# Yachim/schwarzschild-raytracer

Hardware: AMD Instinct MI355X
Metric: Mpixels/s at 1920x1080, 2000 geodesic steps; 1/2/4/8 MI355X (higher is better)
Workload: dtype f32

## Files before the change

schwarzschild-raytracer_amd/csrc/device_scene.h:

```cpp
#ifndef SR_DEVICE_SCENE_H
#define SR_DEVICE_SCENE_H

#include <stdint.h>

#include "sr/sr.h"

#define SR_OBJ_FLOATS 120

#define SR_F_POS 0
#define SR_F_AXES 3
#define SR_F_P0 12
#define SR_F_BOX_FACE0 16
#define SR_F_FACE_STRIDE 14

#define SR_KIND_EXACT 0
#define SR_KIND_BUDGET 1
#define SR_KIND_CHORD 2
#define SR_MU_PLANAR 1.0e-4f
#define SR_MU_QUADRATIC 2.0e-3f
#define SR_CYL_QMARGIN 4.0e-6f
#ifndef SR_BUDGET_DPMIN
#define SR_BUDGET_DPMIN 0.02f
#endif
#ifndef SR_BUDGET_TMAX
// ... 16 lines not shown
    float pl1;
    float f[SR_OBJ_FLOATS - 4];
} sr_dev_obj;

typedef struct {
    int32_t type;
    int32_t cyl;
    float rb, mp, br, mu, pl1;
    float qk;
    float bc[3], x0;
    float pos[3], x1;
    float a0[3], x2;
    float a1[3], rf;
    float a2[3], cn;
} sr_dev_slot;

#define SR_PS_HITS 4
#define SR_PS_FIELDS (4 + 8 * SR_PS_HITS + 16)
#define SR_OPQ_RADIUS 2

#define SR_SEG_FLOATS 16
#define SR_TR_BLOCK 8
#define SR_TR_GROUP 8
#define SR_TR_BLOCKS ((SR_MAX_POINTS - 1 + SR_TR_BLOCK - 1) / SR_TR_BLOCK)
#define SR_TR_GROUPS ((SR_TR_BLOCKS + SR_TR_GROUP - 1) / SR_TR_GROUP)
#define SR_TR_BOUND_FLOATS 12
#define SR_SEGS_BUF_FLOATS ((SR_MAX_POINTS - 1) * SR_SEG_FLOATS + (SR_TR_BLOCKS + SR_TR_GROUPS) * SR_TR_BOUND_FLOATS)

typedef struct {
    int32_t num_objects;
// ... 92 lines not shown
```

schwarzschild-raytracer_amd/csrc/kernels/geodesic.hip:

```cpp
#include <hip/hip_runtime.h>

#include <cstdint>
#include <type_traits>

typedef float sr_v4f __attribute__((ext_vector_type(4)));
typedef const __attribute__((address_space(4))) sr_v4f sr_cfloat4;
__device__ __forceinline__ float4 ldc(const sr_cfloat4* p) {
    const sr_v4f v = *p;
    return make_float4(v.x, v.y, v.z, v.w);
}

#include "../device_scene.h"

namespace {

#define SR_PI 3.1415926535f
#define SR_EPS 0.0000001f

struct f2 { float x, y; };
struct f3 { float x, y, z; };
struct f4 { float x, y, z, w; };
struct m3 { f3 c0, c1, c2; };

__device__ __forceinline__ f2 F2(float x, float y) { f2 r; r.x = x; r.y = y; return r; }
// ... 306 lines not shown
    const float th0 = __builtin_fmaf(kap, len, __builtin_fmaf(2.0f * perr, il, 1e-4f));
    const float m = (sl.mp + sl.mu * __builtin_fmaf(3.1f, a, 1.0f)) * 1.001f + perr;
    const float R = fabsf(y) - m;
    if (!(R > 0.0f)) return 0.0f;
    const float b = c + th0;
    const float L = (__builtin_amdgcn_sqrtf(__builtin_fmaf(b, b, 2.0f * kap * R)) - b) * (a2 * (1.0f / 6.06f));
    const float ch = 1.5f * a * dphi;
    const float Lc = fminf(L, fminf(__builtin_fmaf(0.5f, a, -ch), (1.5f - th0) * (a2 * (1.0f / 6.06f)) - ch));
    const float th1 = __builtin_fmaf(kap, Lc, th0);
    const float f = 1.0f - (th1 * th1 + th1 * th0 + th0 * th0) * (1.0f / 6.0f);
    return (Lc > 0.0f && f > 0.0f) ? Lc * f * 0.998f : 0.0f;
}
#ifndef SR_INIT_WINDOW
#define SR_INIT_WINDOW 1
#endif
__device__ __forceinline__ float plane_window_start(const sr_dev_slot& sl, f3 A, f3 d, float a, float perr, float dphi) {
    const f3 nrm_ = ld3(sl.a1);
    const float y = dot(A - ld3(sl.pos), nrm_);
    if (!(a > 1.0f)) return 0.0f;
    const float a2 = a * a;
    const float kap = 6.06f * __builtin_amdgcn_rcpf(a2);
    const float c = (y > 0.0f ? -1.0f : 1.0f) * dot(d, nrm_);
    const float th0 = 1e-4f;
    const float m = (sl.mp + sl.mu * __builtin_fmaf(3.1f, a, 1.0f)) * 1.001f + perr;
    const float R = fabsf(y) - m;
    if (!(R > 0.0f)) return 0.0f;
    const float b = c + th0;
    const float L = (__builtin_amdgcn_sqrtf(__builtin_fmaf(b, b, 2.0f * kap * R)) - b) * (a2 * (1.0f / 6.06f));
    const float ch = 1.5f * a * dphi;
    const float Lc = fminf(L, fminf(__builtin_fmaf(0.5f, a, -ch), (1.5f - th0) * (a2 * (1.0f / 6.06f)) - ch));
    const float th1 = __builtin_fmaf(kap, Lc, th0);
    const float f = 1.0f - (th1 * th1 + th1 * th0 + th0 * th0) * (1.0f / 6.0f);
    return (Lc > 0.0f && f > 0.0f) ? Lc * f * 0.998f : 0.0f;
}
#ifndef SR_OUT_CYL_CM
#define SR_OUT_CYL_CM 1
#endif
#ifndef SR_OUT_FAR
#define SR_OUT_FAR 1
#endif
__device__ __forceinline__ bool outward_slot(const sr_dev_slot& sl, bool cyl_par, float a, float dip) {
    if (SR_OUT_CYL_CM) cyl_par = false;
    if (sl.type == SR_OBJECT_PLANE || (sl.type == SR_OBJECT_CYLINDER && (cyl_par || !(sl.x1 > 0.0f)))) return false;
    if (SR_OUT_FAR)
        return outward_clear(sl.rf, 0.0f, slot_mu(sl), sl.type == SR_OBJECT_CYLINDER ? sl.qk : 0.0f, sl.pl1, a, dip);
// ... 118 lines not shown
    __device__ __forceinline__ void setMh(float v) const { st(L::BMH, v); }
    __device__ __forceinline__ uint32_t cm() const { return __float_as_uint(ld(L::BCM)) & 0xffu; }
    __device__ __forceinline__ uint32_t excl() const { return __float_as_uint(ld(L::BCM)) >> 8; }
    __device__ __forceinline__ void setCm(uint32_t cm, uint32_t excl) const {
        st(L::BCM, __uint_as_float(cm | (excl << 8)));
    }
    __device__ __forceinline__ float etr() const { return ld(L::BTR); }
    __device__ __forceinline__ void setEtr(float v) const { st(L::BTR, v); }
    __device__ __forceinline__ float uhi() const { return ld(L::BUHI); }
    __device__ __forceinline__ void setUhi(float v) const { st(L::BUHI, v); }
    static __device__ __forceinline__ bool inner(float uhi) { return uhi > SR_BH_U && uhi < 1.0f; }
    static __device__ __forceinline__ float ulo_of(float uhi, float u_f) { return inner(uhi) ? SR_BH_ULO2 : u_f; }
    SR_PROBE_BUDGET_FIELDS
};

__device__ __forceinline__ uint32_t xplane_bit(const sr_dev_slot& sl, int j, f3 n, float nn, float xs) {
    if (sl.type == SR_OBJECT_PLANE || sl.type == SR_OBJECT_CYLINDER) return 0u;
    const float h = dot(ld3(sl.bc), n);
    const float need = (sl.br + sl.mu * xs) * 1.001f + 1.0e-4f + 1.0e-5f * sl.cn;
    return (uint32_t)(h * h > (need * need) * (nn * 1.0002f)) << j;
}
#ifndef SR_XCYL
#define SR_XCYL 1
#endif
__device__ __forceinline__ uint32_t xcyl_bit(const sr_dev_slot& sl, int j, f3 n, float nn, float need) {
    const float h = dot(ld3(sl.bc), n);
    return (uint32_t)(h * h > (need * need) * (nn * 1.0002f)) << j;
}
__device__ __forceinline__ float orbit_e(float u, float du) {
    return u < 0.6f ? __builtin_fmaf(du, du, u * u * (1.0f - u)) : INFINITY;
}
#ifndef SR_XPERI
#define SR_XPERI 1
#endif
template <class BS>
__device__ __forceinline__ uint32_t budget_cyl_frame(const sr_dev_scene* __restrict__ sc, BS& bs, f3 nv, f3 tv) {
    uint32_t c = (uint32_t)sc->budget_cyl_mask;
    uint32_t cm = 0;
#pragma unroll
    for (int k = 0; k < BS::NC; k++) {
        if (c) {
            const f3 ax = ld3(sc->slots[__builtin_ctz(c)].a1);
// ... 24 lines not shown
    }
#endif
    bs.setCm(cm, x);
}

template <class BS>
__device__ __forceinline__ bool cyl_par_bit(const sr_dev_scene* __restrict__ sc, const BS& bs, int j) {
    const uint32_t cyl = (uint32_t)sc->budget_cyl_mask;
    if (!((cyl >> (j - 1)) & 1u)) return false;
    return (bs.cm() >> __builtin_popcount(cyl & ((1u << (j - 1)) - 1u))) & 1u;
}

__device__ float clearance_tr(const sr_dev_scene* __restrict__ sc, const float* __restrict__ segs, f3 A, bool outward,
                              float a, float dip, float rlen, uint32_t& gm);

template <bool START_WINDOW, class BS>
__device__ __forceinline__ void budget_init(const sr_dev_scene* __restrict__ sc, const float* __restrict__ segs,
                                            BS& bs, f3 A, f3 nv, f3 tv,
                                            bool outward, float dip, bool bh_ok, bool falling, float xs, float u2w,
                                            const float* xneed, const float* xperi, float eo, f3 d, float dphi) {
    const float a = __builtin_amdgcn_sqrtf(dot(A, A));
    const int nb = sc->num_budget;
    bs.setT(0.0f);
    bs.setC(dot(A, nv), dot(A, tv));
    const float m0 = 2.0e-6f * (a + 1.0f);
    float m = INFINITY;
    const uint32_t cm = budget_cyl_frame(sc, bs, nv, tv);
    bs.setCm(cm, 0u);
    const f3 xn = cross(nv, tv);
    const float xnn = dot(xn, xn);
    uint32_t xcl = 0;
    {
        float e = clearance_bh(a);
        float uhi = SR_U_NOWIN;
        if (SR_BH_WINDOW && bh_ok && a > SR_BH_RWIN) {
            e = INFINITY;
            uhi = SR_BH_U;
        }
        if (SR_BH_WINDOW2 && dip > SR_BH_DIP2 && a * u2w > 1.000001f && a < SR_BH_RMAX2 && (falling || !(a > SR_BH_RWIN))) {
            e = INFINITY;
            uhi = u2w;
        }
        bs.setUhi(uhi);
        if (outward && outward_clear(1.0f, 0.0f, SR_MU_QUADRATIC, 0.0f, 0.0f, a, dip)) e = INFINITY;
        e -= m0;
        bs.E[0] = e;
        m = nmin(m, e);
    }
    if constexpr (BS::TR) {
        uint32_t gm;
        const float e = clearance_tr(sc, segs, A, outward, a, dip, -1.0f, gm) - m0;
        bs.setEtr(e);
        m = nmin(m, e);
    }
    sr_dev_slot nxt;
    if (nb > 0) nxt = sc->slots[0];
#pragma unroll 1
    for (int j = 1; j <= nb; j++) {
        const sr_dev_slot sl = pin_slot(nxt);
        if (j < nb) nxt = sc->slots[j];
        if (SR_XPLANE) xcl |= xplane_bit(sl, j, xn, xnn, xs);
        if (SR_XCYL && eo <= SR_XCYL_EMAX) xcl |= xcyl_bit(sl, j, xn, xnn, xneed[j - 1]);
        if (SR_XPERI && eo <= xperi[j - 1]) xcl |= 1u << j;
        float e = clearance_obj(sl, A, a) - m0;
        if (START_WINDOW && SR_INIT_WINDOW && (sl.type == SR_OBJECT_RECTANGLE || sl.type == SR_OBJECT_DISK ||
                               sl.type == SR_OBJECT_HOLLOW_DISK || sl.type == SR_OBJECT_PLANE) &&
            sl.mp < INFINITY && e < 0.5f * a) {
            const float w = plane_window_start(sl, A, d, a, m0, dphi);
            e = w > e ? w : e;
        }
        if (outward && outward_slot(sl, cyl_par_bit(sc, bs, j), a, dip)) e = INFINITY;
        if ((xcl >> j) & 1u) e = INFINITY;
        bs.E[j * SR_E_STRIDE] = e;
        m = nmin(m, e);
    }
    bs.setCm(cm, xcl);
    bs.setM(m);
    float mh = INFINITY;
    uint32_t c = (uint32_t)sc->budget_cyl_mask;
#pragma unroll
    for (int k = 0; k < BS::NC; k++) {
        if (c) {
            const float e = clearance_slab(sc->slots[__builtin_ctz(c)], A, a) - m0;
            bs.E[(BS::L::SLAB0 + k) * SR_E_STRIDE] = e;
            mh = nmin(mh, e);
            c &= c - 1;
        }
    }
    bs.setMh(mh);
}

template <int NC>
struct CylDirs {
    float pa[NC > 0 ? NC : 1], pb[NC > 0 ? NC : 1];
};
template <class BS>
__device__ __forceinline__ CylDirs<BS::NC> cyl_dirs(const sr_dev_scene* __restrict__ sc, const BS& bs) {
    CylDirs<BS::NC> d;
// ... 940 lines not shown
        return F4(at(f, id), at(f + 1, id), at(f + 2, id), at(f + 3, id));
    }
};

__device__ __forceinline__ f4 crosshair_frag(const sr_dev_frame& fr, const Pix& q) {
    f4 frag = F4(0.0f, 0.0f, 0.0f, 0.0f);
    if (fr.crosshair) {
        f2 uv = F2((float)(2 * q.px + 1) / (float)fr.width - 1.0f, (float)(2 * q.py + 1) / (float)fr.height - 1.0f);
        float hx = fabsf(uv.x * fr.res_x / 2.0f), hy = fabsf(uv.y * fr.res_y / 2.0f);
        if ((hx < 1.0f && hy > 5.0f && hy < 15.0f) || (hy < 1.0f && hx > 5.0f && hx < 15.0f))
            frag = F4(0.5f, 0.5f, 0.5f, 0.5f);
    }
    return frag;
}

__device__ __forceinline__ int init_pixel(const sr_dev_frame& fr, const sr_dev_cam& cam, const Pix& q, Ray& r) {
    f2 uv = F2((float)(2 * q.px + 1) / (float)fr.width - 1.0f, (float)(2 * q.py + 1) / (float)fr.height - 1.0f);
    f2 uvv = F2(uv.x, uv.y * fr.res_y / fr.res_x);
    m3 axes = ldm(cam.axes);
    r.ro = ld3(cam.pos);
    r.rd = nrm(mv(axes, F3(uvv.x, uvv.y, cam.ray_forward)));
    r.nv = nrm(r.ro);
    r.steps = 0;
    r.i = 0;
    SR_PROBE(probe_ray_init(r));
    const bool flat = fr.raytrace_type == SR_RAYTRACE_FLAT ||
                      (fr.raytrace_type == SR_RAYTRACE_HALF_WIDTH && uv.x > 2.0f * fr.curved_percentage + -1.0f) ||
                      (fr.raytrace_type == SR_RAYTRACE_HALF_HEIGHT && uv.y > 2.0f * fr.curved_percentage + -1.0f);
    if (flat || fabsf(dot(r.rd, r.nv)) >= 1.0f - SR_EPS) return ST_FLAT;
    if (fr.percent_black >= 0.0f) {
        float x = t_sin(uvv.x * 12.9898f + uvv.y * 78.233f) * 43758.5453f;
        if (x - floorf(x) <= fr.percent_black) return ST_DONE;
    }
    r.tv = nrm(cross(cross(r.nv, r.rd), r.nv));
    r.u = 1.0f / len(r.ro);
    r.du = -r.u * dot(r.rd, r.nv) / dot(r.rd, r.tv);
    return -1;
}

__shared__ uint32_t sr_lds_pid[SR_WG];
struct HitLog {
    PS ps;
    int n;
    __device__ __forceinline__ uint32_t id() const {
        typedef volatile const __attribute__((address_space(3))) uint32_t lds_u32;
        uint32_t t = threadIdx.x;
        asm volatile("" : "+v"(t));
        return *(lds_u32*)&sr_lds_pid[t];
    }
};
// ... 20 lines not shown
    const float l4 = ddu(u + k3 * h);
    un = u + h6 * (__builtin_fmaf(2.0f, k3, __builtin_fmaf(2.0f, k2, k1)) + k4);
    dun = du + h6 * (__builtin_fmaf(2.0f, l3, __builtin_fmaf(2.0f, l2, l1)) + l4);
}

__device__ __forceinline__ bool flat_misses(const sr_dev_scene* __restrict__ sc, f3 ro, f3 rd) {
    return !sc->tr_visible && dot(ro, rd) >= 0.0f && dot(ro, ro) > sc->flat_miss_r2;
}

__shared__ int sr_lds_ev[SR_WG / 64];

template <bool CULL, bool RECORD, bool WCOST = false, int NB = SR_MAX_BUDGET, int FU = SR_FAST_UNROLL,
          int NC = SR_NC_KERNEL, bool TR = false>
__device__ __forceinline__ int integrate(const sr_dev_scene* __restrict__ sc, const float* __restrict__ segs,
                                         const float4* __restrict__ tbl, const sr_dev_frame& fr, const Tex& tx,
                                         Ray& r, Hit& hit, HitLog& log) {
    using BS = Budget<NB, NC, TR && CULL>;
    __shared__ float lds_E[BS::L::ROWS * SR_E_STRIDE];
    BS bs;
    bs.E = lds_E + threadIdx.x;
    SR_PROBE(SR_PROF_CLOCK(prof_bi_));
    if (!CULL) bs.setUhi(INFINITY);
    if (CULL)
        budget_init<RECORD>(sc, segs, bs, r.ro, r.nv, r.tv, r.du < 0.0f && r.u < 0.6f, fr.out_dip,
                            fr.win_ok && fr.out_dip > SR_BH_DIP, r.du > 0.0f, fr.xplane_s, fr.bh_u2, fr.xlow_need,
                            fr.xperi_e, orbit_e(r.u, r.du), r.rd, fr.max_dphi);
    SR_PROBE(FireProbe<Ray, BS> fire_probe_(r, bs));
    const int N = fr.max_steps;
    const bool every = !CULL || sc->num_step > 0 || (sc->tr_visible && !BS::TR);
    int im = r.i - 1;
    float up = 0.0f;
    float rA = __builtin_amdgcn_rcpf(r.u);
    const int sbase = r.steps - r.i;
    auto phi_cs = [&](int j) -> f2 {
        if (j < 0) return F2(1.0f, 0.0f);
        const float4 t = tbl[j];
        return F2(t.z, t.w);
    };
    auto settle_prev = [&](int i) {
        if (im == i - 1) return;
        const f2 p1 = phi_cs(i - 1);
// ... 361 lines not shown
#define SR_SPLIT 0x80

__device__ __forceinline__ int split_thread(int sub, int tid, int lg) {
    const int lane = tid & 63;
    if (lane >= (1 << lg)) return -1;
    const int cell = sub * 4 + (tid >> 6);
    const int side = lg >> 1;
    const int cpq = 64 >> lg;
    const int quad = cell / cpq, qc = cell % cpq;
    const int per_row = 8 >> side;
    const int x8 = ((qc % per_row) << side) + (lane & ((1 << side) - 1));
    const int y8 = ((qc / per_row) << side) + (lane >> side);
    return quad * 64 + y8 * 8 + x8;
}

template <bool CULL, bool WCOST = false, int NB = SR_MAX_BUDGET, int FU = SR_FAST_UNROLL, int NC = SR_NC_KERNEL,
          bool TR = false>
__global__ __launch_bounds__(SR_WG, sr_integrate_waves(NB, NC)) void sr_integrate_kernel(
    const sr_dev_scene* __restrict__ sc, const float4* __restrict__ tbl, const float* __restrict__ segs,
    const uint32_t* __restrict__ arr, const uint8_t* __restrict__ opq, sr_dev_frame fr, float* __restrict__ ps_base,
    size_t ps_n, int* __restrict__ count, const int* __restrict__ order, int* __restrict__ cost) {
    const unsigned B = (unsigned)fr.batch;
    const unsigned bid = blockIdx.x;
    const unsigned wg = bid / SR_WG_PER_TILE;
    const int frame = B > 1 ? (int)(wg % B) : 0;
    const unsigned slot = B > 1 ? wg / B : wg;
    const int code = order ? order[slot] : ((int)slot << 8);
    if (blockIdx.x == 0 && threadIdx.x == 0) *count = 0;
    if (code < 0) return;
    const int block = code >> 8;
    const int ttid = (int)(bid % SR_WG_PER_TILE) * SR_WG + (int)threadIdx.x;
    const int tid = (code & SR_SPLIT) ? split_thread(code & 0x3f, ttid, fr.split_log2) : ttid;
#ifndef SR_PRIO_BLOCKS
#define SR_PRIO_BLOCKS 256
#endif
#ifdef SR_PRIO_SPLIT
// ... 3 lines not shown
#endif
    SR_PROBE(WaveProbe wp);
    Pix q;
    int steps = 0;
    if (WCOST && (threadIdx.x & 63) == 0) sr_lds_ev[threadIdx.x >> 6] = 0;
    if (tid >= 0 && pixel_of(fr, block, tid, q)) {
        sr_lds_pid[threadIdx.x] = (uint32_t)(((size_t)frame * (size_t)fr.tiles + (size_t)block) * 256 + tid);
        Tex tx;
        tx.bg = nullptr;
        tx.arr = arr;
        tx.opq = opq;
        HitLog log{PS{ps_base, ps_n}, 0};
        const PS& ps = log.ps;
        Ray r;
        Hit hit;
        int st = init_pixel(fr, fr.cam[frame], q, r);
        SR_PROBE(st = wp.lane_mask(q.px, q.py, fr.width, st, ST_DONE); wp.ray_start(r));
        if (st < 0) st = integrate<CULL, true, WCOST, NB, FU, NC, TR>(sc, segs, tbl, fr, tx, r, hit, log);
        const size_t id = log.id();
        ps.put_rec(id, ps_word(st, log.n, r.steps), r.rd);
        SR_PROBE(wp.pixel(st, log.n));
        if (st == ST_FLAT || st == ST_MORE) ps.put3(PS_RO, id, r.ro);
        if (st == ST_MORE) {
            ps.puti(PS_I, id, r.i);
            ps.put3(PS_NV, id, r.nv);
            ps.put3(PS_TV, id, r.tv);
            ps.at(PS_U, id) = r.u;
            ps.at(PS_DU, id) = r.du;
        }
        steps = r.steps;
        SR_PROBE(wp.ray_end(r));
    }
    SR_PROBE(wp.finish(frame, fr.tiles, block, ttid, steps));
// ... 193 lines not shown
        }
        const size_t fo = (size_t)f * (size_t)fr.width * (size_t)fr.nrows;
        write_pixel(fr, out ? out + (size_t)f * (size_t)fr.out_frame_stride : nullptr, pitch,
                    dbg_rgba ? dbg_rgba + 4 * fo : nullptr, dbg_steps ? dbg_steps + fo : nullptr, q, frag, r.steps);
        if (fr.wave_cost) {
            const int nb8 = (fr.nrows + 7) >> 3, nc8 = (fr.width + 7) >> 3;
            atomicMax(fr.wave_cost + (((size_t)f * nb8 + (q.k >> 3)) * nc8 + (q.px >> 3)) * 2, r.steps);
        }
    }
}

extern "C" hipError_t sr_launch_geodesic(const sr_dev_scene* sc, const float4* tbl, const float* segs,
                                         const uint32_t* bg, const uint32_t* arr, const uint8_t* opq,
                                         const sr_dev_frame* fr, uint8_t* out, size_t pitch, float* dbg_rgba,
                                         int32_t* dbg_steps, float* ps, size_t ps_n, int* list, int* count,
                                         int* order, int* cost, int* diag, hipEvent_t* ev4, hipStream_t stream) {
    dim3 block(256);
    dim3 grid((fr->width + 15) / 16, (fr->nrows + 15) / 16);
    if (grid.x == 0 || grid.y == 0) return hipSuccess;
    const unsigned nblocks = grid.x * grid.y;
    const unsigned B = (unsigned)fr->batch;
    if (B < 1 || B > SR_MAX_BATCH || fr->tiles != (int)nblocks) return hipErrorInvalidValue;
    if ((size_t)nblocks * B * 256 > ps_n || (size_t)nblocks * B * 256 > (size_t)INT32_MAX) return hipErrorInvalidValue;
    if ((order == nullptr) != (cost == nullptr)) return hipErrorInvalidValue;
    const int split = order ? fr->split_tiles : 0;
    if (split < 0 || (split && (fr->split_log2 < 0 || fr->split_log2 > 4 || (fr->split_log2 & 1))))
        return hipErrorInvalidValue;
    if (nblocks > (1u << 22)) return hipErrorInvalidValue;
    const unsigned slots = nblocks + ((64u >> (split ? fr->split_log2 : 6)) - 1u) * (unsigned)split;
    const bool cull = fr->cull != 0;
    const bool small = cull && fr->num_budget <= SR_NB_SMALL && fr->num_budget_cyl <= SR_NC_SMALL;
    const bool general = fr->num_budget <= SR_NB_GENERAL;
    const bool tr = cull && fr->tr_visible != 0;
    if (cull && fr->num_budget_cyl > SR_NC_KERNEL && !small) return hipErrorInvalidValue;
    if (ev4) (void)hipEventRecord(ev4[0], stream);
    if (fr->wave_cost && general)
        hipLaunchKernelGGL((sr_integrate_kernel<true, true, SR_NB_GENERAL, SR_FAST_UNROLL, SR_NC_GENERAL>),
                           dim3(slots * B * SR_WG_PER_TILE), dim3(SR_WG), 0, stream,
                           sc, tbl, segs, arr, opq, *fr, ps, ps_n, count, order, cost);
    else if (fr->wave_cost)
        hipLaunchKernelGGL((sr_integrate_kernel<true, true>), dim3(slots * B * SR_WG_PER_TILE), dim3(SR_WG), 0, stream,
                           sc, tbl, segs, arr, opq, *fr, ps, ps_n, count, order, cost);
    else if (small && tr)
        hipLaunchKernelGGL((sr_integrate_kernel<true, false, SR_NB_SMALL, SR_FAST_UNROLL, SR_NC_SMALL, true>),
                           dim3(slots * B * SR_WG_PER_TILE), dim3(SR_WG), 0, stream, sc, tbl, segs, arr, opq, *fr, ps,
                           ps_n, count, order, cost);
    else if (cull && general && tr)
        hipLaunchKernelGGL((sr_integrate_kernel<true, false, SR_NB_GENERAL, SR_FAST_UNROLL, SR_NC_GENERAL, true>),
                           dim3(slots * B * SR_WG_PER_TILE), dim3(SR_WG), 0, stream, sc, tbl, segs, arr, opq, *fr, ps,
                           ps_n, count, order, cost);
    else if (cull && tr)
        hipLaunchKernelGGL((sr_integrate_kernel<true, false, SR_MAX_BUDGET, SR_FAST_UNROLL, SR_NC_KERNEL, true>),
                           dim3(slots * B * SR_WG_PER_TILE), dim3(SR_WG), 0, stream, sc, tbl, segs, arr, opq, *fr, ps,
                           ps_n, count, order, cost);
    else if (small && fr->fast_unroll == 2)
        hipLaunchKernelGGL((sr_integrate_kernel<true, false, SR_NB_SMALL, 2, SR_NC_SMALL>), dim3(slots * B * SR_WG_PER_TILE),
                           dim3(SR_WG), 0, stream, sc, tbl, segs, arr, opq, *fr, ps, ps_n, count, order, cost);
    else if (small)
        hipLaunchKernelGGL((sr_integrate_kernel<true, false, SR_NB_SMALL, SR_FAST_UNROLL, SR_NC_SMALL>),
                           dim3(slots * B * SR_WG_PER_TILE),
                           dim3(SR_WG), 0, stream, sc, tbl, segs, arr, opq, *fr, ps, ps_n, count, order, cost);
    else if (cull && general)
        hipLaunchKernelGGL((sr_integrate_kernel<true, false, SR_NB_GENERAL, SR_FAST_UNROLL, SR_NC_GENERAL>),
                           dim3(slots * B * SR_WG_PER_TILE), dim3(SR_WG), 0, stream, sc,
                           tbl, segs, arr, opq, *fr, ps, ps_n, count, order, cost);
    else if (cull)
        hipLaunchKernelGGL(sr_integrate_kernel<true>, dim3(slots * B * SR_WG_PER_TILE), dim3(SR_WG), 0, stream, sc,
                           tbl, segs, arr, opq, *fr, ps, ps_n, count, order, cost);
    else
        hipLaunchKernelGGL((sr_integrate_kernel<false, false, 1, SR_FAST_UNROLL, 1>), dim3(slots * B * SR_WG_PER_TILE),
                           dim3(SR_WG), 0, stream, sc, tbl, segs, arr, opq, *fr, ps, ps_n, count, order, cost);
    if (ev4) (void)hipEventRecord(ev4[1], stream);
    OrderArgs oa{cost, order, (int)nblocks, fr->max_steps, split, split ? fr->split_log2 : 6, fr->split_min_steps};
    hipLaunchKernelGGL(sr_shade_kernel, dim3(grid.x, grid.y * B + (order ? 1u : 0u)), block, 0, stream, sc, segs, bg,
                       arr, *fr, ps, ps_n, out, pitch, dbg_rgba, dbg_steps, list, count, diag, oa);
    if (ev4) (void)hipEventRecord(ev4[2], stream);
#ifndef SR_RESUME_TILES
#define SR_RESUME_TILES 1024u
#endif
    unsigned nb = (nblocks * B < SR_RESUME_TILES ? nblocks * B : SR_RESUME_TILES) * SR_WG_PER_TILE;
    if (tr)
        hipLaunchKernelGGL((sr_resume_kernel<true, true>), dim3(nb), dim3(SR_WG), 0, stream, sc, tbl, segs, bg, arr, *fr,
                           ps, ps_n, out, pitch, dbg_rgba, dbg_steps, list, count);
    else if (cull)
        hipLaunchKernelGGL(sr_resume_kernel<true>, dim3(nb), dim3(SR_WG), 0, stream, sc, tbl, segs, bg, arr, *fr, ps, ps_n,
                           out, pitch, dbg_rgba, dbg_steps, list, count);
// ... 7 lines not shown
```

schwarzschild-raytracer_amd/csrc/sr_api.cpp:

```cpp
#include <hip/hip_runtime.h>

#include <algorithm>
#include <array>
#include <cmath>
#include <cstdio>
#include <cstring>
#include <map>
#include <new>
#include <tuple>
#include <utility>
#include <vector>

#include "device_scene.h"
#include "sr/sr.h"

#ifndef SR_CYL_DIRFREE
#define SR_CYL_DIRFREE 1
#endif

extern "C" hipError_t sr_launch_geodesic(const sr_dev_scene* sc, const float4* tbl, const float* segs,
                                         const uint32_t* bg, const uint32_t* arr, const uint8_t* opq,
                                         const sr_dev_frame* fr,
                                         uint8_t* out, size_t pitch, float* dbg_rgba, int32_t* dbg_steps,
                                         float* ps, size_t ps_n, int* list, int* count, int* order, int* cost,
                                         int* diag, hipEvent_t* ev4, hipStream_t stream);

namespace {

constexpr float kPi = 3.1415926535f;

struct Table {
    float4* dev = nullptr;
    int steps = 0;
    std::vector<float4> host;
    uint64_t used = 0;
};

constexpr size_t kCacheEntries = 8;

}
// ... 28 lines not shown
        int* dev = nullptr;
        uint64_t used = 0;
    };
    std::map<std::vector<int>, BlockList> block_lists;
    uint64_t tick = 0;
    hipStream_t upload = nullptr;
    int split_tiles = 0, split_log2 = 4, split_min_steps = 1;
    int fast_unroll = SR_FAST_UNROLL_DEFAULT;
    const int* last_order = nullptr;
    size_t last_slots = 0;
    hipStream_t last_stream = nullptr;
    bool launched = false;
    hipEvent_t order_ev = nullptr;
    int64_t free_errors = 0;
    int* d_diag = nullptr;
    std::vector<hipEvent_t> tev;
    int timing_cap = 0;
    int timing_n = 0;
    std::map<std::pair<int, int>, Table> tables;
};

namespace {

struct V3 {
    float x, y, z;
};
inline V3 v3(float x, float y, float z) { return {x, y, z}; }
inline V3 ld(const float* p) { return {p[0], p[1], p[2]}; }
inline void st(float* p, V3 v) {
    p[0] = v.x;
// ... 737 lines not shown
    rc = ensure_table(ctx, params->max_steps, params->max_revolutions, s, &tbl);
    if (rc != SR_OK) return rc;
    rc = ensure_pixel_state(ctx, (size_t)fr.tiles * (size_t)n_frames * 256, s);
    if (rc != SR_OK) return rc;
    int* order = nullptr;
    int* cost = nullptr;
    if (nrows > 0) {
        rc = ensure_order(ctx, (width + 15) / 16, (nrows + 15) / 16, d_block_list, s, &order, &cost);
        if (rc != SR_OK) return rc;
        ctx->last_order = order;
        ctx->last_slots = (size_t)((width + 15) / 16) * (size_t)((nrows + 15) / 16) +
                          (size_t)((64 >> (ctx->split_tiles ? ctx->split_log2 : 6)) - 1) * (size_t)ctx->split_tiles;
    }
    hipError_t e = sr_launch_geodesic(ctx->d_scene, tbl, ctx->d_segs, ctx->d_bg, ctx->d_arr, ctx->d_opq, &fr, out, pitch,
                                      dbg_rgba, dbg_steps, ctx->d_ps, ctx->ps_n, ctx->d_list, ctx->d_count, order, cost,
                                      ctx->d_diag,
                                      ctx->timing_n < ctx->timing_cap ? &ctx->tev[4 * (size_t)ctx->timing_n++] : nullptr,
                                      s);
    if (hip_ok(e)) e = hipEventRecord(ctx->order_ev, s);
    ctx->launched = true;
    return hip_ok(e) ? SR_OK : SR_E_HIP;
}

}

extern "C" hipError_t sr_assemble_blocks_device(const uint8_t* stacked, size_t rank_stride, size_t in_frame_stride,
                                                const int* dev_lists, int world, int per, int height, int block_rows,
                                                size_t row_bytes, uint8_t* out, size_t out_frame_stride, int n_frames,
                                                hipStream_t stream);
extern "C" int sr_assemble_blocks_host(const uint8_t* stacked, size_t rank_stride, size_t in_frame_stride,
                                       const int* lists, int world, int per, int height, int block_rows,
// ... 44 lines not shown
    c->device = hip_device;
    std::memset(&c->h_scene, 0, sizeof c->h_scene);
    c->h_scene.flat_miss_r2 = INFINITY;
    if (!hip_ok(hipStreamCreateWithFlags(&c->upload, hipStreamNonBlocking))) {
        c->upload = nullptr;
        sr_destroy(c);
        return SR_E_HIP;
    }
    if (!hip_ok(hipEventCreateWithFlags(&c->order_ev, hipEventDisableTiming))) {
        c->order_ev = nullptr;
        sr_destroy(c);
        return SR_E_HIP;
    }
    if (!hip_ok(hipMalloc(&c->d_scene, sizeof(sr_dev_scene))) ||
        !hip_ok(hipMalloc(&c->d_segs, (size_t)SR_SEGS_BUF_FLOATS * sizeof(float))) ||
        !hip_ok(hipMalloc(reinterpret_cast<void**>(&c->d_diag), sizeof(int)))) {
        sr_destroy(c);
        return SR_E_NOMEM;
    }
    if (!hip_ok(hipMemsetAsync(c->d_scene, 0, sizeof(sr_dev_scene), c->upload)) ||
        !hip_ok(hipMemsetAsync(c->d_diag, 0, sizeof(int), c->upload)) ||
        !hip_ok(hipMemsetAsync(c->d_segs, 0, (size_t)SR_SEGS_BUF_FLOATS * sizeof(float),
                               c->upload)) ||
        !hip_ok(hipStreamSynchronize(c->upload))) {
        sr_destroy(c);
        return SR_E_HIP;
    }
    sr_test_ray tr;
    sr_test_ray_default(&tr);
    int rc = sr_set_test_ray(c, &tr);
    if (rc != SR_OK) {
        sr_destroy(c);
        return rc;
    }
    *out = c;
    return SR_OK;
}

void sr_destroy(sr_ctx* c) {
    if (!c) return;
    (void)hipSetDevice(c->device);
    (void)wait_ctx(c);
    if (c->d_scene) (void)hipFree(c->d_scene);
    if (c->d_segs) (void)hipFree(c->d_segs);
    if (c->d_diag) (void)hipFree(c->d_diag);
    const hipStream_t s = c->upload;
    if (s) {
        c->launched = false;
        release(c, c->d_bg, s);
        release(c, c->d_arr, s);
        release(c, c->d_opq, s);
        for (auto& kv : c->tables) release(c, kv.second.dev, s);
        free_pixel_state(c, s);
        for (auto& kv : c->orders) {
            release(c, kv.second.order, s);
            release(c, kv.second.cost, s);
        }
        for (auto& kv : c->block_lists) release(c, kv.second.dev, s);
        (void)hipStreamSynchronize(s);
        (void)hipStreamDestroy(s);
// ... 429 lines not shown
```

Baseline: 2801.

## Precompute per-camera start clearances in a table kernel before integration

Adds a small kernel that, once per frame and camera, computes the ray-origin-dependent clearance values: black-hole start bounds, test-ray clearance for both outward states, per-slot object clearance, plane-window parameters and slab clearances. The integrate kernel's budget initialisation then reads this table instead of recomputing the same camera-only work for every pixel, leaving only direction-dependent terms per ray. The cost is an extra serial single-thread launch and loads from a global table, and the design relies on outward_slot no longer depending on per-ray state.

```diff
diff --git a/schwarzschild-raytracer_amd/csrc/device_scene.h b/schwarzschild-raytracer_amd/csrc/device_scene.h
--- a/schwarzschild-raytracer_amd/csrc/device_scene.h
+++ b/schwarzschild-raytracer_amd/csrc/device_scene.h
@@ -54,6 +54,33 @@
     float a1[3], rf;
     float a2[3], cn;
 } sr_dev_slot;
+
+#define SR_START_CYL 4
+#define SR_START_OUT 1
+#define SR_START_WIN 2
+typedef struct {
+    float e;
+    float k2r;
+    float need;
+    int32_t flags;
+    float bc[3];
+    float xneed;
+    float wn[3];
+    float xperi;
+} sr_dev_start_slot;
+typedef struct {
+    float nv[3];
+    float u;
+    float a;
+    float cx;
+    float e_bh[2];
+    float uhi[2];
+    float e_tr[2];
+    int32_t bh_out;
+    float kap, a2s, cap;
+    float slab[SR_START_CYL];
+    sr_dev_start_slot slot[SR_MAX_BUDGET];
+} sr_dev_start;
 
 #define SR_PS_HITS 4
 #define SR_PS_FIELDS (4 + 8 * SR_PS_HITS + 16)
diff --git a/schwarzschild-raytracer_amd/csrc/kernels/geodesic.hip b/schwarzschild-raytracer_amd/csrc/kernels/geodesic.hip
--- a/schwarzschild-raytracer_amd/csrc/kernels/geodesic.hip
+++ b/schwarzschild-raytracer_amd/csrc/kernels/geodesic.hip
@@ -344,21 +344,41 @@
 #ifndef SR_INIT_WINDOW
 #define SR_INIT_WINDOW 1
 #endif
-__device__ __forceinline__ float plane_window_start(const sr_dev_slot& sl, f3 A, f3 d, float a, float perr, float dphi) {
+struct PlaneWinCam {
+    bool ok;
+    f3 wn;
+    float k2r;
+    float kap, a2s, cap;
+};
+__device__ __forceinline__ PlaneWinCam plane_window_cam(const sr_dev_slot& sl, f3 A, float a, float perr, float dphi) {
+    PlaneWinCam w;
+    w.ok = false;
+    w.wn = F3(0.0f, 0.0f, 0.0f);
+    w.k2r = w.kap = w.a2s = w.cap = 0.0f;
     const f3 nrm_ = ld3(sl.a1);
     const float y = dot(A - ld3(sl.pos), nrm_);
-    if (!(a > 1.0f)) return 0.0f;
+    if (!(a > 1.0f)) return w;
     const float a2 = a * a;
     const float kap = 6.06f * __builtin_amdgcn_rcpf(a2);
-    const float c = (y > 0.0f ? -1.0f : 1.0f) * dot(d, nrm_);
+    w.wn = nrm_ * (y > 0.0f ? -1.0f : 1.0f);
     const float th0 = 1e-4f;
     const float m = (sl.mp + sl.mu * __builtin_fmaf(3.1f, a, 1.0f)) * 1.001f + perr;
     const float R = fabsf(y) - m;
-    if (!(R > 0.0f)) return 0.0f;
+    if (!(R > 0.0f)) return w;
+    w.k2r = 2.0f * kap * R;
+    w.kap = kap;
+    w.a2s = a2 * (1.0f / 6.06f);
+    const float ch = 1.5f * a * dphi;
+    w.cap = fminf(__builtin_fmaf(0.5f, a, -ch), (1.5f - th0) * (a2 * (1.0f / 6.06f)) - ch);
+    w.ok = true;
+    return w;
+}
+__device__ __forceinline__ float plane_window_dir(f3 wn, float k2r, float kap, float a2s, float cap, f3 d) {
+    const float c = dot(d, wn);
+    const float th0 = 1e-4f;
     const float b = c + th0;
-    const float L = (__builtin_amdgcn_sqrtf(__builtin_fmaf(b, b, 2.0f * kap * R)) - b) * (a2 * (1.0f / 6.06f));
-    const float ch = 1.5f * a * dphi;
-    const float Lc = fminf(L, fminf(__builtin_fmaf(0.5f, a, -ch), (1.5f - th0) * (a2 * (1.0f / 6.06f)) - ch));
+    const float L = (__builtin_amdgcn_sqrtf(__builtin_fmaf(b, b, k2r)) - b) * a2s;
+    const float Lc = fminf(L, cap);
     const float th1 = __builtin_fmaf(kap, Lc, th0);
     const float f = 1.0f - (th1 * th1 + th1 * th0 + th0 * th0) * (1.0f / 6.0f);
     return (Lc > 0.0f && f > 0.0f) ? Lc * f * 0.998f : 0.0f;
@@ -507,18 +527,22 @@
     SR_PROBE_BUDGET_FIELDS
 };
 
+__device__ __forceinline__ float xplane_need(const sr_dev_slot& sl, float xs) {
+    if (sl.type == SR_OBJECT_PLANE || sl.type == SR_OBJECT_CYLINDER) return INFINITY;
+    return (sl.br + sl.mu * xs) * 1.001f + 1.0e-4f + 1.0e-5f * sl.cn;
+}
+__device__ __forceinline__ uint32_t plane_off_bit(f3 bc, int j, f3 n, float nn, float need) {
+    const float h = dot(bc, n);
+    return (uint32_t)(h * h > (need * need) * (nn * 1.0002f)) << j;
+}
 __device__ __forceinline__ uint32_t xplane_bit(const sr_dev_slot& sl, int j, f3 n, float nn, float xs) {
-    if (sl.type == SR_OBJECT_PLANE || sl.type == SR_OBJECT_CYLINDER) return 0u;
-    const float h = dot(ld3(sl.bc), n);
-    const float need = (sl.br + sl.mu * xs) * 1.001f + 1.0e-4f + 1.0e-5f * sl.cn;
-    return (uint32_t)(h * h > (need * need) * (nn * 1.0002f)) << j;
+    return plane_off_bit(ld3(sl.bc), j, n, nn, xplane_need(sl, xs));
 }
 #ifndef SR_XCYL
 #define SR_XCYL 1
 #endif
 __device__ __forceinline__ uint32_t xcyl_bit(const sr_dev_slot& sl, int j, f3 n, float nn, float need) {
-    const float h = dot(ld3(sl.bc), n);
-    return (uint32_t)(h * h > (need * need) * (nn * 1.0002f)) << j;
+    return plane_off_bit(ld3(sl.bc), j, n, nn, need);
 }
 __device__ __forceinline__ float orbit_e(float u, float du) {
     return u < 0.6f ? __builtin_fmaf(du, du, u * u * (1.0f - u)) : INFINITY;
@@ -573,11 +597,25 @@
 __device__ float clearance_tr(const sr_dev_scene* __restrict__ sc, const float* __restrict__ segs, f3 A, bool outward,
                               float a, float dip, float rlen, uint32_t& gm);
 
-template <bool START_WINDOW, class BS>
+__device__ __forceinline__ float bh_start(float a, float dip, bool bh_ok, bool falling, float u2w, float& uhi) {
+    float e = clearance_bh(a);
+    uhi = SR_U_NOWIN;
+    if (SR_BH_WINDOW && bh_ok && a > SR_BH_RWIN) {
+        e = INFINITY;
+        uhi = SR_BH_U;
+    }
+    if (SR_BH_WINDOW2 && dip > SR_BH_DIP2 && a * u2w > 1.000001f && a < SR_BH_RMAX2 && (falling || !(a > SR_BH_RWIN))) {
+        e = INFINITY;
+        uhi = u2w;
+    }
+    return e;
+}
+
+template <class BS>
 __device__ __forceinline__ void budget_init(const sr_dev_scene* __restrict__ sc, const float* __restrict__ segs,
                                             BS& bs, f3 A, f3 nv, f3 tv,
                                             bool outward, float dip, bool bh_ok, bool falling, float xs, float u2w,
-                                            const float* xneed, const float* xperi, float eo, f3 d, float dphi) {
+                                            const float* xneed, const float* xperi, float eo) {
     const float a = __builtin_amdgcn_sqrtf(dot(A, A));
     const int nb = sc->num_budget;
     bs.setT(0.0f);
@@ -590,16 +628,8 @@
     const float xnn = dot(xn, xn);
     uint32_t xcl = 0;
     {
-        float e = clearance_bh(a);
-        float uhi = SR_U_NOWIN;
-        if (SR_BH_WINDOW && bh_ok && a > SR_BH_RWIN) {
-            e = INFINITY;
-            uhi = SR_BH_U;
-        }
-        if (SR_BH_WINDOW2 && dip > SR_BH_DIP2 && a * u2w > 1.000001f && a < SR_BH_RMAX2 && (falling || !(a > SR_BH_RWIN))) {
-            e = INFINITY;
-            uhi = u2w;
-        }
+        float uhi;
+        float e = bh_start(a, dip, bh_ok, falling, u2w, uhi);
         bs.setUhi(uhi);
         if (outward && outward_clear(1.0f, 0.0f, SR_MU_QUADRATIC, 0.0f, 0.0f, a, dip)) e = INFINITY;
         e -= m0;
@@ -622,12 +652,6 @@
         if (SR_XCYL && eo <= SR_XCYL_EMAX) xcl |= xcyl_bit(sl, j, xn, xnn, xneed[j - 1]);
         if (SR_XPERI && eo <= xperi[j - 1]) xcl |= 1u << j;
         float e = clearance_obj(sl, A, a) - m0;
-        if (START_WINDOW && SR_INIT_WINDOW && (sl.type == SR_OBJECT_RECTANGLE || sl.type == SR_OBJECT_DISK ||
-                               sl.type == SR_OBJECT_HOLLOW_DISK || sl.type == SR_OBJECT_PLANE) &&
-            sl.mp < INFINITY && e < 0.5f * a) {
-            const float w = plane_window_start(sl, A, d, a, m0, dphi);
-            e = w > e ? w : e;
-        }
         if (outward && outward_slot(sl, cyl_par_bit(sc, bs, j), a, dip)) e = INFINITY;
         if ((xcl >> j) & 1u) e = INFINITY;
         bs.E[j * SR_E_STRIDE] = e;
@@ -641,6 +665,170 @@
     for (int k = 0; k < BS::NC; k++) {
         if (c) {
             const float e = clearance_slab(sc->slots[__builtin_ctz(c)], A, a) - m0;
+            bs.E[(BS::L::SLAB0 + k) * SR_E_STRIDE] = e;
+            mh = nmin(mh, e);
+            c &= c - 1;
+        }
+    }
+    bs.setMh(mh);
+}
+
+static_assert(SR_OUT_CYL_CM == 1, "the start table holds outward_slot per camera: keep cyl_par per ray otherwise");
+__device__ void build_start(const sr_dev_scene* __restrict__ sc, const float* __restrict__ segs, const sr_dev_frame& fr,
+                            f3 A, sr_dev_start& o) {
+    const f3 nv = nrm(A);
+    o.nv[0] = nv.x;
+    o.nv[1] = nv.y;
+    o.nv[2] = nv.z;
+    o.u = 1.0f / len(A);
+    const float a = __builtin_amdgcn_sqrtf(dot(A, A));
+    const float m0 = 2.0e-6f * (a + 1.0f);
+    const float dip = fr.out_dip;
+    o.a = a;
+    o.cx = dot(A, nv);
+    for (int falling = 0; falling < 2; falling++) {
+        float uhi;
+        const float e = bh_start(a, dip, fr.win_ok && fr.out_dip > SR_BH_DIP, falling != 0, fr.bh_u2, uhi);
+        o.e_bh[falling] = e - m0;
+        o.uhi[falling] = uhi;
+    }
+    o.bh_out = outward_clear(1.0f, 0.0f, SR_MU_QUADRATIC, 0.0f, 0.0f, a, dip) ? 1 : 0;
+    for (int outward = 0; outward < 2; outward++) {
+        uint32_t gm;
+        o.e_tr[outward] = fr.tr_visible ? clearance_tr(sc, segs, A, outward != 0, a, dip, -1.0f, gm) - m0 : 0.0f;
+    }
+    o.kap = o.a2s = o.cap = 0.0f;
+    int nb = sc->num_budget;
+    nb = nb < SR_MAX_BUDGET ? nb : SR_MAX_BUDGET;
+    for (int j = 0; j < nb; j++) {
+        const sr_dev_slot& sl = sc->slots[j];
+        sr_dev_start_slot& t = o.slot[j];
+        float e = clearance_obj(sl, A, a) - m0;
+        int flags = 0;
+        f3 wn = F3(0.0f, 0.0f, 0.0f);
+        float k2r = 0.0f;
+        if (SR_INIT_WINDOW && (sl.type == SR_OBJECT_RECTANGLE || sl.type == SR_OBJECT_DISK ||
+                               sl.type == SR_OBJECT_HOLLOW_DISK || sl.type == SR_OBJECT_PLANE) &&
+            sl.mp < INFINITY && e < 0.5f * a) {
+            const PlaneWinCam w = plane_window_cam(sl, A, a, m0, fr.max_dphi);
+            if (w.ok) {
+                flags |= SR_START_WIN;
+                wn = w.wn;
+                k2r = w.k2r;
+                o.kap = w.kap;
+                o.a2s = w.a2s;
+                o.cap = w.cap;
+            } else {
+                const float w0 = 0.0f;
+                e = w0 > e ? w0 : e;
+            }
+        }
+        if (outward_slot(sl, false, a, dip)) flags |= SR_START_OUT;
+        t.e = e;
+        t.k2r = k2r;
+        t.need = SR_XPLANE ? xplane_need(sl, fr.xplane_s) : INFINITY;
+        t.flags = flags;
+        t.bc[0] = sl.bc[0];
+        t.bc[1] = sl.bc[1];
+        t.bc[2] = sl.bc[2];
+        t.xneed = fr.xlow_need[j];
+        t.wn[0] = wn.x;
+        t.wn[1] = wn.y;
+        t.wn[2] = wn.z;
+        t.xperi = fr.xperi_e[j];
+    }
+    uint32_t c = (uint32_t)sc->budget_cyl_mask;
+    for (int k = 0; k < SR_START_CYL; k++) {
+        o.slab[k] = INFINITY;
+        if (c) {
+            o.slab[k] = clearance_slab(sc->slots[__builtin_ctz(c)], A, a) - m0;
+            c &= c - 1;
+        }
+    }
+}
+
+__device__ __forceinline__ sr_dev_start_slot pin_start_slot(const sr_dev_start_slot& g) {
+    sr_dev_start_slot t = g;
+    SR_PIN(t.e);
+    SR_PIN(t.k2r);
+    SR_PIN(t.need);
+    SR_PIN(t.flags);
+    SR_PIN(t.bc[0]);
+    SR_PIN(t.bc[1]);
+    SR_PIN(t.bc[2]);
+    SR_PIN(t.xneed);
+    SR_PIN(t.wn[0]);
+    SR_PIN(t.wn[1]);
+    SR_PIN(t.wn[2]);
+    SR_PIN(t.xperi);
+    return t;
+}
+
+template <class BS>
+__device__ __forceinline__ void budget_start(const sr_dev_scene* __restrict__ sc, const sr_dev_start& st, BS& bs, int nb,
+                                             f3 A, f3 nv, f3 tv, bool outward, bool falling, float eo, f3 d) {
+    static_assert(BS::NC <= SR_START_CYL, "sr_dev_start.slab holds SR_START_CYL cylinders");
+    sr_dev_start_slot nxt;
+    if (nb > 0) nxt = st.slot[0];
+    bs.setT(0.0f);
+    bs.setC(st.cx, dot(A, tv));
+    float m = INFINITY;
+    const uint32_t cm = budget_cyl_frame(sc, bs, nv, tv);
+    const f3 xn = cross(nv, tv);
+    const float xnn = dot(xn, xn);
+    uint32_t xcl = 0;
+    float e0 = st.e_bh[0], e1 = st.e_bh[1], uh0 = st.uhi[0], uh1 = st.uhi[1];
+    float kap = st.kap, a2s = st.a2s, cap = st.cap;
+    int bh_out = st.bh_out;
+    SR_PIN(e0);
+    SR_PIN(e1);
+    SR_PIN(uh0);
+    SR_PIN(uh1);
+    SR_PIN(kap);
+    SR_PIN(a2s);
+    SR_PIN(cap);
+    SR_PIN(bh_out);
+    {
+        float e = falling ? e1 : e0;
+        bs.setUhi(falling ? uh1 : uh0);
+        if (outward && bh_out) e = INFINITY;
+        bs.E[0] = e;
+        m = nmin(m, e);
+    }
+    if constexpr (BS::TR) {
+        float t0 = st.e_tr[0], t1 = st.e_tr[1];
+        SR_PIN(t0);
+        SR_PIN(t1);
+        const float e = outward ? t1 : t0;
+        bs.setEtr(e);
+        m = nmin(m, e);
+    }
+#pragma unroll 1
+    for (int j = 1; j <= nb; j++) {
+        const sr_dev_start_slot t = pin_start_slot(nxt);
+        if (j < nb) nxt = st.slot[j];
+        const f3 bc = ld3(t.bc);
+        if (SR_XPLANE) xcl |= plane_off_bit(bc, j, xn, xnn, t.need);
+        if (SR_XCYL && eo <= SR_XCYL_EMAX) xcl |= plane_off_bit(bc, j, xn, xnn, t.xneed);
+        if (SR_XPERI && eo <= t.xperi) xcl |= 1u << j;
+        float e = t.e;
+        if (t.flags & SR_START_WIN) {
+            const float w = plane_window_dir(ld3(t.wn), t.k2r, kap, a2s, cap, d);
+            e = w > e ? w : e;
+        }
+        if (outward && (t.flags & SR_START_OUT)) e = INFINITY;
+        if ((xcl >> j) & 1u) e = INFINITY;
+        bs.E[j * SR_E_STRIDE] = e;
+        m = nmin(m, e);
+    }
+    bs.setCm(cm, xcl);
+    bs.setM(m);
+    float mh = INFINITY;
+    uint32_t c = (uint32_t)sc->budget_cyl_mask;
+#pragma unroll
+    for (int k = 0; k < BS::NC; k++) {
+        if (c) {
+            const float e = st.slab[k];
             bs.E[(BS::L::SLAB0 + k) * SR_E_STRIDE] = e;
             mh = nmin(mh, e);
             c &= c - 1;
@@ -1611,13 +1799,14 @@
     return frag;
 }
 
-__device__ __forceinline__ int init_pixel(const sr_dev_frame& fr, const sr_dev_cam& cam, const Pix& q, Ray& r) {
+__device__ __forceinline__ int init_pixel(const sr_dev_frame& fr, const sr_dev_cam& cam, const sr_dev_start& st,
+                                          const Pix& q, Ray& r) {
     f2 uv = F2((float)(2 * q.px + 1) / (float)fr.width - 1.0f, (float)(2 * q.py + 1) / (float)fr.height - 1.0f);
     f2 uvv = F2(uv.x, uv.y * fr.res_y / fr.res_x);
     m3 axes = ldm(cam.axes);
     r.ro = ld3(cam.pos);
     r.rd = nrm(mv(axes, F3(uvv.x, uvv.y, cam.ray_forward)));
-    r.nv = nrm(r.ro);
+    r.nv = ld3(st.nv);
     r.steps = 0;
     r.i = 0;
     SR_PROBE(probe_ray_init(r));
@@ -1630,7 +1819,7 @@
         if (x - floorf(x) <= fr.percent_black) return ST_DONE;
     }
     r.tv = nrm(cross(cross(r.nv, r.rd), r.nv));
-    r.u = 1.0f / len(r.ro);
+    r.u = st.u;
     r.du = -r.u * dot(r.rd, r.nv) / dot(r.rd, r.tv);
     return -1;
 }
@@ -1681,17 +1870,20 @@
           int NC = SR_NC_KERNEL, bool TR = false>
 __device__ __forceinline__ int integrate(const sr_dev_scene* __restrict__ sc, const float* __restrict__ segs,
                                          const float4* __restrict__ tbl, const sr_dev_frame& fr, const Tex& tx,
-                                         Ray& r, Hit& hit, HitLog& log) {
+                                         Ray& r, Hit& hit, HitLog& log, const sr_dev_start* __restrict__ start = nullptr) {
     using BS = Budget<NB, NC, TR && CULL>;
     __shared__ float lds_E[BS::L::ROWS * SR_E_STRIDE];
     BS bs;
     bs.E = lds_E + threadIdx.x;
     SR_PROBE(SR_PROF_CLOCK(prof_bi_));
     if (!CULL) bs.setUhi(INFINITY);
-    if (CULL)
-        budget_init<RECORD>(sc, segs, bs, r.ro, r.nv, r.tv, r.du < 0.0f && r.u < 0.6f, fr.out_dip,
-                            fr.win_ok && fr.out_dip > SR_BH_DIP, r.du > 0.0f, fr.xplane_s, fr.bh_u2, fr.xlow_need,
-                            fr.xperi_e, orbit_e(r.u, r.du), r.rd, fr.max_dphi);
+    if constexpr (CULL && RECORD)
+        budget_start(sc, *start, bs, fr.num_budget, r.ro, r.nv, r.tv, r.du < 0.0f && r.u < 0.6f, r.du > 0.0f,
+                     orbit_e(r.u, r.du), r.rd);
+    else if (CULL)
+        budget_init(sc, segs, bs, r.ro, r.nv, r.tv, r.du < 0.0f && r.u < 0.6f, fr.out_dip,
+                    fr.win_ok && fr.out_dip > SR_BH_DIP, r.du > 0.0f, fr.xplane_s, fr.bh_u2, fr.xlow_need,
+                    fr.xperi_e, orbit_e(r.u, r.du));
     SR_PROBE(FireProbe<Ray, BS> fire_probe_(r, bs));
     const int N = fr.max_steps;
     const bool every = !CULL || sc->num_step > 0 || (sc->tr_visible && !BS::TR);
@@ -2083,12 +2275,21 @@
     return quad * 64 + y8 * 8 + x8;
 }
 
+__global__ __launch_bounds__(64) void sr_start_table_kernel(const sr_dev_scene* __restrict__ sc,
+                                                            const float* __restrict__ segs, sr_dev_frame fr,
+                                                            sr_dev_start* __restrict__ start) {
+    const int f = (int)blockIdx.x;
+    if (f >= fr.batch || threadIdx.x != 0) return;
+    build_start(sc, segs, fr, ld3(fr.cam[f].pos), start[f]);
+}
+
 template <bool CULL, bool WCOST = false, int NB = SR_MAX_BUDGET, int FU = SR_FAST_UNROLL, int NC = SR_NC_KERNEL,
           bool TR = false>
 __global__ __launch_bounds__(SR_WG, sr_integrate_waves(NB, NC)) void sr_integrate_kernel(
     const sr_dev_scene* __restrict__ sc, const float4* __restrict__ tbl, const float* __restrict__ segs,
     const uint32_t* __restrict__ arr, const uint8_t* __restrict__ opq, sr_dev_frame fr, float* __restrict__ ps_base,
-    size_t ps_n, int* __restrict__ count, const int* __restrict__ order, int* __restrict__ cost) {
+    size_t ps_n, int* __restrict__ count, const int* __restrict__ order, int* __restrict__ cost,
+    const sr_dev_start* __restrict__ start) {
     const unsigned B = (unsigned)fr.batch;
     const unsigned bid = blockIdx.x;
     const unsigned wg = bid / SR_WG_PER_TILE;
@@ -2122,9 +2323,9 @@
         const PS& ps = log.ps;
         Ray r;
         Hit hit;
-        int st = init_pixel(fr, fr.cam[frame], q, r);
+        int st = init_pixel(fr, fr.cam[frame], start[frame], q, r);
         SR_PROBE(st = wp.lane_mask(q.px, q.py, fr.width, st, ST_DONE); wp.ray_start(r));
-        if (st < 0) st = integrate<CULL, true, WCOST, NB, FU, NC, TR>(sc, segs, tbl, fr, tx, r, hit, log);
+        if (st < 0) st = integrate<CULL, true, WCOST, NB, FU, NC, TR>(sc, segs, tbl, fr, tx, r, hit, log, start + frame);
         const size_t id = log.id();
         ps.put_rec(id, ps_word(st, log.n, r.steps), r.rd);
         SR_PROBE(wp.pixel(st, log.n));
@@ -2348,7 +2549,8 @@
                                          const uint32_t* bg, const uint32_t* arr, const uint8_t* opq,
                                          const sr_dev_frame* fr, uint8_t* out, size_t pitch, float* dbg_rgba,
                                          int32_t* dbg_steps, float* ps, size_t ps_n, int* list, int* count,
-                                         int* order, int* cost, int* diag, hipEvent_t* ev4, hipStream_t stream) {
+                                         int* order, int* cost, int* diag, sr_dev_start* start, hipEvent_t* ev4,
+                                         hipStream_t stream) {
     dim3 block(256);
     dim3 grid((fr->width + 15) / 16, (fr->nrows + 15) / 16);
     if (grid.x == 0 || grid.y == 0) return hipSuccess;
@@ -2367,43 +2569,45 @@
     const bool general = fr->num_budget <= SR_NB_GENERAL;
     const bool tr = cull && fr->tr_visible != 0;
     if (cull && fr->num_budget_cyl > SR_NC_KERNEL && !small) return hipErrorInvalidValue;
+    if (!start) return hipErrorInvalidValue;
     if (ev4) (void)hipEventRecord(ev4[0], stream);
+    hipLaunchKernelGGL(sr_start_table_kernel, dim3(B), dim3(1), 0, stream, sc, segs, *fr, start);
     if (fr->wave_cost && general)
         hipLaunchKernelGGL((sr_integrate_kernel<true, true, SR_NB_GENERAL, SR_FAST_UNROLL, SR_NC_GENERAL>),
                            dim3(slots * B * SR_WG_PER_TILE), dim3(SR_WG), 0, stream,
-                           sc, tbl, segs, arr, opq, *fr, ps, ps_n, count, order, cost);
+                           sc, tbl, segs, arr, opq, *fr, ps, ps_n, count, order, cost, start);
     else if (fr->wave_cost)
         hipLaunchKernelGGL((sr_integrate_kernel<true, true>), dim3(slots * B * SR_WG_PER_TILE), dim3(SR_WG), 0, stream,
-                           sc, tbl, segs, arr, opq, *fr, ps, ps_n, count, order, cost);
+                           sc, tbl, segs, arr, opq, *fr, ps, ps_n, count, order, cost, start);
     else if (small && tr)
         hipLaunchKernelGGL((sr_integrate_kernel<true, false, SR_NB_SMALL, SR_FAST_UNROLL, SR_NC_SMALL, true>),
                            dim3(slots * B * SR_WG_PER_TILE), dim3(SR_WG), 0, stream, sc, tbl, segs, arr, opq, *fr, ps,
-                           ps_n, count, order, cost);
+                           ps_n, count, order, cost, start);
     else if (cull && general && tr)
         hipLaunchKernelGGL((sr_integrate_kernel<true, false, SR_NB_GENERAL, SR_FAST_UNROLL, SR_NC_GENERAL, true>),
                            dim3(slots * B * SR_WG_PER_TILE), dim3(SR_WG), 0, stream, sc, tbl, segs, arr, opq, *fr, ps,
-                           ps_n, count, order, cost);
+                           ps_n, count, order, cost, start);
     else if (cull && tr)
         hipLaunchKernelGGL((sr_integrate_kernel<true, false, SR_MAX_BUDGET, SR_FAST_UNROLL, SR_NC_KERNEL, true>),
                            dim3(slots * B * SR_WG_PER_TILE), dim3(SR_WG), 0, stream, sc, tbl, segs, arr, opq, *fr, ps,
-                           ps_n, count, order, cost);
+                           ps_n, count, order, cost, start);
     else if (small && fr->fast_unroll == 2)
         hipLaunchKernelGGL((sr_integrate_kernel<true, false, SR_NB_SMALL, 2, SR_NC_SMALL>), dim3(slots * B * SR_WG_PER_TILE),
-                           dim3(SR_WG), 0, stream, sc, tbl, segs, arr, opq, *fr, ps, ps_n, count, order, cost);
+                           dim3(SR_WG), 0, stream, sc, tbl, segs, arr, opq, *fr, ps, ps_n, count, order, cost, start);
     else if (small)
         hipLaunchKernelGGL((sr_integrate_kernel<true, false, SR_NB_SMALL, SR_FAST_UNROLL, SR_NC_SMALL>),
                            dim3(slots * B * SR_WG_PER_TILE),
-                           dim3(SR_WG), 0, stream, sc, tbl, segs, arr, opq, *fr, ps, ps_n, count, order, cost);
+                           dim3(SR_WG), 0, stream, sc, tbl, segs, arr, opq, *fr, ps, ps_n, count, order, cost, start);
     else if (cull && general)
         hipLaunchKernelGGL((sr_integrate_kernel<true, false, SR_NB_GENERAL, SR_FAST_UNROLL, SR_NC_GENERAL>),
                            dim3(slots * B * SR_WG_PER_TILE), dim3(SR_WG), 0, stream, sc,
-                           tbl, segs, arr, opq, *fr, ps, ps_n, count, order, cost);
+                           tbl, segs, arr, opq, *fr, ps, ps_n, count, order, cost, start);
     else if (cull)
         hipLaunchKernelGGL(sr_integrate_kernel<true>, dim3(slots * B * SR_WG_PER_TILE), dim3(SR_WG), 0, stream, sc,
-                           tbl, segs, arr, opq, *fr, ps, ps_n, count, order, cost);
+                           tbl, segs, arr, opq, *fr, ps, ps_n, count, order, cost, start);
     else
         hipLaunchKernelGGL((sr_integrate_kernel<false, false, 1, SR_FAST_UNROLL, 1>), dim3(slots * B * SR_WG_PER_TILE),
-                           dim3(SR_WG), 0, stream, sc, tbl, segs, arr, opq, *fr, ps, ps_n, count, order, cost);
+                           dim3(SR_WG), 0, stream, sc, tbl, segs, arr, opq, *fr, ps, ps_n, count, order, cost, start);
     if (ev4) (void)hipEventRecord(ev4[1], stream);
     OrderArgs oa{cost, order, (int)nblocks, fr->max_steps, split, split ? fr->split_log2 : 6, fr->split_min_steps};
     hipLaunchKernelGGL(sr_shade_kernel, dim3(grid.x, grid.y * B + (order ? 1u : 0u)), block, 0, stream, sc, segs, bg,
diff --git a/schwarzschild-raytracer_amd/csrc/sr_api.cpp b/schwarzschild-raytracer_amd/csrc/sr_api.cpp
--- a/schwarzschild-raytracer_amd/csrc/sr_api.cpp
+++ b/schwarzschild-raytracer_amd/csrc/sr_api.cpp
@@ -23,7 +23,7 @@
                                          const sr_dev_frame* fr,
                                          uint8_t* out, size_t pitch, float* dbg_rgba, int32_t* dbg_steps,
                                          float* ps, size_t ps_n, int* list, int* count, int* order, int* cost,
-                                         int* diag, hipEvent_t* ev4, hipStream_t stream);
+                                         int* diag, sr_dev_start* start, hipEvent_t* ev4, hipStream_t stream);
 
 namespace {
 
@@ -82,6 +82,7 @@
     hipEvent_t order_ev = nullptr;
     int64_t free_errors = 0;
     int* d_diag = nullptr;
+    sr_dev_start* d_start = nullptr;
     std::vector<hipEvent_t> tev;
     int timing_cap = 0;
     int timing_n = 0;
@@ -849,7 +850,7 @@
     }
     hipError_t e = sr_launch_geodesic(ctx->d_scene, tbl, ctx->d_segs, ctx->d_bg, ctx->d_arr, ctx->d_opq, &fr, out, pitch,
                                       dbg_rgba, dbg_steps, ctx->d_ps, ctx->ps_n, ctx->d_list, ctx->d_count, order, cost,
-                                      ctx->d_diag,
+                                      ctx->d_diag, ctx->d_start,
                                       ctx->timing_n < ctx->timing_cap ? &ctx->tev[4 * (size_t)ctx->timing_n++] : nullptr,
                                       s);
     if (hip_ok(e)) e = hipEventRecord(ctx->order_ev, s);
@@ -924,12 +925,14 @@
     }
     if (!hip_ok(hipMalloc(&c->d_scene, sizeof(sr_dev_scene))) ||
         !hip_ok(hipMalloc(&c->d_segs, (size_t)SR_SEGS_BUF_FLOATS * sizeof(float))) ||
-        !hip_ok(hipMalloc(reinterpret_cast<void**>(&c->d_diag), sizeof(int)))) {
+        !hip_ok(hipMalloc(reinterpret_cast<void**>(&c->d_diag), sizeof(int))) ||
+        !hip_ok(hipMalloc(reinterpret_cast<void**>(&c->d_start), SR_MAX_BATCH * sizeof(sr_dev_start)))) {
         sr_destroy(c);
         return SR_E_NOMEM;
     }
     if (!hip_ok(hipMemsetAsync(c->d_scene, 0, sizeof(sr_dev_scene), c->upload)) ||
         !hip_ok(hipMemsetAsync(c->d_diag, 0, sizeof(int), c->upload)) ||
+        !hip_ok(hipMemsetAsync(c->d_start, 0, SR_MAX_BATCH * sizeof(sr_dev_start), c->upload)) ||
         !hip_ok(hipMemsetAsync(c->d_segs, 0, (size_t)SR_SEGS_BUF_FLOATS * sizeof(float),
                                c->upload)) ||
         !hip_ok(hipStreamSynchronize(c->upload))) {
@@ -954,6 +957,7 @@
     if (c->d_scene) (void)hipFree(c->d_scene);
     if (c->d_segs) (void)hipFree(c->d_segs);
     if (c->d_diag) (void)hipFree(c->d_diag);
+    if (c->d_start) (void)hipFree(c->d_start);
     const hipStream_t s = c->upload;
     if (s) {
         c->launched = false;
```

Result: faster. 2861 (median of 6 runs) (+2.2%).
